# jialeli1/From-Voxel-to-Point

Measured on AMD Instinct MI355X. Metric: point clouds/sec fwd+bwd (FV2P, KITTI shape) at 1/2/4/8 MI355X, higher is better.
Workload: dtype f32

## Files before the change

### from-voxel-to-point_amd/csrc/sa_fused.hip

```cpp
#include "common.hpp"

namespace fv2p {

typedef float f32x4 __attribute__((ext_vector_type(4)));

constexpr int kSaC = 64;
constexpr int kSaCentres = 16;

__device__ __forceinline__ void row16_max_n(float (&v)[16]) {
  asm volatile(
      "s_nop 1\n\t"
      "v_max_f32_dpp %0, %0, %0 quad_perm:[1,0,3,2] row_mask:0xf bank_mask:0xf\n\t"
      "v_max_f32_dpp %1, %1, %1 quad_perm:[1,0,3,2] row_mask:0xf bank_mask:0xf\n\t"
      "v_max_f32_dpp %2, %2, %2 quad_perm:[1,0,3,2] row_mask:0xf bank_mask:0xf\n\t"
      "v_max_f32_dpp %3, %3, %3 quad_perm:[1,0,3,2] row_mask:0xf bank_mask:0xf\n\t"
      "v_max_f32_dpp %4, %4, %4 quad_perm:[1,0,3,2] row_mask:0xf bank_mask:0xf\n\t"
      "v_max_f32_dpp %5, %5, %5 quad_perm:[1,0,3,2] row_mask:0xf bank_mask:0xf\n\t"
      "v_max_f32_dpp %6, %6, %6 quad_perm:[1,0,3,2] row_mask:0xf bank_mask:0xf\n\t"
      "v_max_f32_dpp %7, %7, %7 quad_perm:[1,0,3,2] row_mask:0xf bank_mask:0xf\n\t"
      "v_max_f32_dpp %8, %8, %8 quad_perm:[1,0,3,2] row_mask:0xf bank_mask:0xf\n\t"
      "v_max_f32_dpp %9, %9, %9 quad_perm:[1,0,3,2] row_mask:0xf bank_mask:0xf\n\t"
      "v_max_f32_dpp %10, %10, %10 quad_perm:[1,0,3,2] row_mask:0xf bank_mask:0xf\n\t"
      "v_max_f32_dpp %11, %11, %11 quad_perm:[1,0,3,2] row_mask:0xf bank_mask:0xf\n\t"
      "v_max_f32_dpp %12, %12, %12 quad_perm:[1,0,3,2] row_mask:0xf bank_mask:0xf\n\t"
      "v_max_f32_dpp %13, %13, %13 quad_perm:[1,0,3,2] row_mask:0xf bank_mask:0xf\n\t"
      "v_max_f32_dpp %14, %14, %14 quad_perm:[1,0,3,2] row_mask:0xf bank_mask:0xf\n\t"
      "v_max_f32_dpp %15, %15, %15 quad_perm:[1,0,3,2] row_mask:0xf bank_mask:0xf\n\t"
      "v_max_f32_dpp %0, %0, %0 quad_perm:[2,3,0,1] row_mask:0xf bank_mask:0xf\n\t"
      "v_max_f32_dpp %1, %1, %1 quad_perm:[2,3,0,1] row_mask:0xf bank_mask:0xf\n\t"
      "v_max_f32_dpp %2, %2, %2 quad_perm:[2,3,0,1] row_mask:0xf bank_mask:0xf\n\t"
      "v_max_f32_dpp %3, %3, %3 quad_perm:[2,3,0,1] row_mask:0xf bank_mask:0xf\n\t"
      "v_max_f32_dpp %4, %4, %4 quad_perm:[2,3,0,1] row_mask:0xf bank_mask:0xf\n\t"
      "v_max_f32_dpp %5, %5, %5 quad_perm:[2,3,0,1] row_mask:0xf bank_mask:0xf\n\t"
      "v_max_f32_dpp %6, %6, %6 quad_perm:[2,3,0,1] row_mask:0xf bank_mask:0xf\n\t"
      "v_max_f32_dpp %7, %7, %7 quad_perm:[2,3,0,1] row_mask:0xf bank_mask:0xf\n\t"
      "v_max_f32_dpp %8, %8, %8 quad_perm:[2,3,0,1] row_mask:0xf bank_mask:0xf\n\t"
      "v_max_f32_dpp %9, %9, %9 quad_perm:[2,3,0,1] row_mask:0xf bank_mask:0xf\n\t"
      "v_max_f32_dpp %10, %10, %10 quad_perm:[2,3,0,1] row_mask:0xf bank_mask:0xf\n\t"
      "v_max_f32_dpp %11, %11, %11 quad_perm:[2,3,0,1] row_mask:0xf bank_mask:0xf\n\t"
      "v_max_f32_dpp %12, %12, %12 quad_perm:[2,3,0,1] row_mask:0xf bank_mask:0xf\n\t"
      "v_max_f32_dpp %13, %13, %13 quad_perm:[2,3,0,1] row_mask:0xf bank_mask:0xf\n\t"
      "v_max_f32_dpp %14, %14, %14 quad_perm:[2,3,0,1] row_mask:0xf bank_mask:0xf\n\t"
      "v_max_f32_dpp %15, %15, %15 quad_perm:[2,3,0,1] row_mask:0xf bank_mask:0xf\n\t"
      "v_max_f32_dpp %0, %0, %0 row_half_mirror row_mask:0xf bank_mask:0xf\n\t"
      "v_max_f32_dpp %1, %1, %1 row_half_mirror row_mask:0xf bank_mask:0xf\n\t"
      "v_max_f32_dpp %2, %2, %2 row_half_mirror row_mask:0xf bank_mask:0xf\n\t"
      "v_max_f32_dpp %3, %3, %3 row_half_mirror row_mask:0xf bank_mask:0xf\n\t"
      "v_max_f32_dpp %4, %4, %4 row_half_mirror row_mask:0xf bank_mask:0xf\n\t"
      "v_max_f32_dpp %5, %5, %5 row_half_mirror row_mask:0xf bank_mask:0xf\n\t"
      "v_max_f32_dpp %6, %6, %6 row_half_mirror row_mask:0xf bank_mask:0xf\n\t"
      "v_max_f32_dpp %7, %7, %7 row_half_mirror row_mask:0xf bank_mask:0xf\n\t"
      "v_max_f32_dpp %8, %8, %8 row_half_mirror row_mask:0xf bank_mask:0xf\n\t"
      "v_max_f32_dpp %9, %9, %9 row_half_mirror row_mask:0xf bank_mask:0xf\n\t"
      "v_max_f32_dpp %10, %10, %10 row_half_mirror row_mask:0xf bank_mask:0xf\n\t"
      "v_max_f32_dpp %11, %11, %11 row_half_mirror row_mask:0xf bank_mask:0xf\n\t"
      "v_max_f32_dpp %12, %12, %12 row_half_mirror row_mask:0xf bank_mask:0xf\n\t"
      "v_max_f32_dpp %13, %13, %13 row_half_mirror row_mask:0xf bank_mask:0xf\n\t"
      "v_max_f32_dpp %14, %14, %14 row_half_mirror row_mask:0xf bank_mask:0xf\n\t"
      "v_max_f32_dpp %15, %15, %15 row_half_mirror row_mask:0xf bank_mask:0xf\n\t"
      "v_max_f32_dpp %0, %0, %0 row_mirror row_mask:0xf bank_mask:0xf\n\t"
      "v_max_f32_dpp %1, %1, %1 row_mirror row_mask:0xf bank_mask:0xf\n\t"
      "v_max_f32_dpp %2, %2, %2 row_mirror row_mask:0xf bank_mask:0xf\n\t"
      "v_max_f32_dpp %3, %3, %3 row_mirror row_mask:0xf bank_mask:0xf\n\t"
      "v_max_f32_dpp %4, %4, %4 row_mirror row_mask:0xf bank_mask:0xf\n\t"
      "v_max_f32_dpp %5, %5, %5 row_mirror row_mask:0xf bank_mask:0xf\n\t"
      "v_max_f32_dpp %6, %6, %6 row_mirror row_mask:0xf bank_mask:0xf\n\t"
      "v_max_f32_dpp %7, %7, %7 row_mirror row_mask:0xf bank_mask:0xf\n\t"
      "v_max_f32_dpp %8, %8, %8 row_mirror row_mask:0xf bank_mask:0xf\n\t"
      "v_max_f32_dpp %9, %9, %9 row_mirror row_mask:0xf bank_mask:0xf\n\t"
      "v_max_f32_dpp %10, %10, %10 row_mirror row_mask:0xf bank_mask:0xf\n\t"
      "v_max_f32_dpp %11, %11, %11 row_mirror row_mask:0xf bank_mask:0xf\n\t"
      "v_max_f32_dpp %12, %12, %12 row_mirror row_mask:0xf bank_mask:0xf\n\t"
      "v_max_f32_dpp %13, %13, %13 row_mirror row_mask:0xf bank_mask:0xf\n\t"
      "v_max_f32_dpp %14, %14, %14 row_mirror row_mask:0xf bank_mask:0xf\n\t"
      "v_max_f32_dpp %15, %15, %15 row_mirror row_mask:0xf bank_mask:0xf\n\t"
      "s_nop 1"
      : "+v"(v[0]), "+v"(v[1]), "+v"(v[2]), "+v"(v[3]), "+v"(v[4]), "+v"(v[5]), "+v"(v[6]), "+v"(v[7]), "+v"(v[8]), "+v"(v[9]), "+v"(v[10]), "+v"(v[11]), "+v"(v[12]), "+v"(v[13]), "+v"(v[14]), "+v"(v[15]));
}
__device__ __forceinline__ void row16_sum_n(float (&v)[16]) {
  asm volatile(
      "s_nop 1\n\t"
      "v_add_f32_dpp %0, %0, %0 quad_perm:[1,0,3,2] row_mask:0xf bank_mask:0xf\n\t"
      "v_add_f32_dpp %1, %1, %1 quad_perm:[1,0,3,2] row_mask:0xf bank_mask:0xf\n\t"
      "v_add_f32_dpp %2, %2, %2 quad_perm:[1,0,3,2] row_mask:0xf bank_mask:0xf\n\t"
      "v_add_f32_dpp %3, %3, %3 quad_perm:[1,0,3,2] row_mask:0xf bank_mask:0xf\n\t"
      "v_add_f32_dpp %4, %4, %4 quad_perm:[1,0,3,2] row_mask:0xf bank_mask:0xf\n\t"
      "v_add_f32_dpp %5, %5, %5 quad_perm:[1,0,3,2] row_mask:0xf bank_mask:0xf\n\t"
      "v_add_f32_dpp %6, %6, %6 quad_perm:[1,0,3,2] row_mask:0xf bank_mask:0xf\n\t"
      "v_add_f32_dpp %7, %7, %7 quad_perm:[1,0,3,2] row_mask:0xf bank_mask:0xf\n\t"
      "v_add_f32_dpp %8, %8, %8 quad_perm:[1,0,3,2] row_mask:0xf bank_mask:0xf\n\t"
      "v_add_f32_dpp %9, %9, %9 quad_perm:[1,0,3,2] row_mask:0xf bank_mask:0xf\n\t"
      "v_add_f32_dpp %10, %10, %10 quad_perm:[1,0,3,2] row_mask:0xf bank_mask:0xf\n\t"
      "v_add_f32_dpp %11, %11, %11 quad_perm:[1,0,3,2] row_mask:0xf bank_mask:0xf\n\t"
      "v_add_f32_dpp %12, %12, %12 quad_perm:[1,0,3,2] row_mask:0xf bank_mask:0xf\n\t"
      "v_add_f32_dpp %13, %13, %13 quad_perm:[1,0,3,2] row_mask:0xf bank_mask:0xf\n\t"
      "v_add_f32_dpp %14, %14, %14 quad_perm:[1,0,3,2] row_mask:0xf bank_mask:0xf\n\t"
      "v_add_f32_dpp %15, %15, %15 quad_perm:[1,0,3,2] row_mask:0xf bank_mask:0xf\n\t"
      "v_add_f32_dpp %0, %0, %0 quad_perm:[2,3,0,1] row_mask:0xf bank_mask:0xf\n\t"
      "v_add_f32_dpp %1, %1, %1 quad_perm:[2,3,0,1] row_mask:0xf bank_mask:0xf\n\t"
      "v_add_f32_dpp %2, %2, %2 quad_perm:[2,3,0,1] row_mask:0xf bank_mask:0xf\n\t"
      "v_add_f32_dpp %3, %3, %3 quad_perm:[2,3,0,1] row_mask:0xf bank_mask:0xf\n\t"
      "v_add_f32_dpp %4, %4, %4 quad_perm:[2,3,0,1] row_mask:0xf bank_mask:0xf\n\t"
      "v_add_f32_dpp %5, %5, %5 quad_perm:[2,3,0,1] row_mask:0xf bank_mask:0xf\n\t"
      "v_add_f32_dpp %6, %6, %6 quad_perm:[2,3,0,1] row_mask:0xf bank_mask:0xf\n\t"
      "v_add_f32_dpp %7, %7, %7 quad_perm:[2,3,0,1] row_mask:0xf bank_mask:0xf\n\t"
      "v_add_f32_dpp %8, %8, %8 quad_perm:[2,3,0,1] row_mask:0xf bank_mask:0xf\n\t"
      "v_add_f32_dpp %9, %9, %9 quad_perm:[2,3,0,1] row_mask:0xf bank_mask:0xf\n\t"
      "v_add_f32_dpp %10, %10, %10 quad_perm:[2,3,0,1] row_mask:0xf bank_mask:0xf\n\t"
      "v_add_f32_dpp %11, %11, %11 quad_perm:[2,3,0,1] row_mask:0xf bank_mask:0xf\n\t"
      "v_add_f32_dpp %12, %12, %12 quad_perm:[2,3,0,1] row_mask:0xf bank_mask:0xf\n\t"
      "v_add_f32_dpp %13, %13, %13 quad_perm:[2,3,0,1] row_mask:0xf bank_mask:0xf\n\t"
      "v_add_f32_dpp %14, %14, %14 quad_perm:[2,3,0,1] row_mask:0xf bank_mask:0xf\n\t"
      "v_add_f32_dpp %15, %15, %15 quad_perm:[2,3,0,1] row_mask:0xf bank_mask:0xf\n\t"
      "v_add_f32_dpp %0, %0, %0 row_half_mirror row_mask:0xf bank_mask:0xf\n\t"
      "v_add_f32_dpp %1, %1, %1 row_half_mirror row_mask:0xf bank_mask:0xf\n\t"
      "v_add_f32_dpp %2, %2, %2 row_half_mirror row_mask:0xf bank_mask:0xf\n\t"
      "v_add_f32_dpp %3, %3, %3 row_half_mirror row_mask:0xf bank_mask:0xf\n\t"
      "v_add_f32_dpp %4, %4, %4 row_half_mirror row_mask:0xf bank_mask:0xf\n\t"
      "v_add_f32_dpp %5, %5, %5 row_half_mirror row_mask:0xf bank_mask:0xf\n\t"
      "v_add_f32_dpp %6, %6, %6 row_half_mirror row_mask:0xf bank_mask:0xf\n\t"
      "v_add_f32_dpp %7, %7, %7 row_half_mirror row_mask:0xf bank_mask:0xf\n\t"
      "v_add_f32_dpp %8, %8, %8 row_half_mirror row_mask:0xf bank_mask:0xf\n\t"
      "v_add_f32_dpp %9, %9, %9 row_half_mirror row_mask:0xf bank_mask:0xf\n\t"
      "v_add_f32_dpp %10, %10, %10 row_half_mirror row_mask:0xf bank_mask:0xf\n\t"
      "v_add_f32_dpp %11, %11, %11 row_half_mirror row_mask:0xf bank_mask:0xf\n\t"
      "v_add_f32_dpp %12, %12, %12 row_half_mirror row_mask:0xf bank_mask:0xf\n\t"
      "v_add_f32_dpp %13, %13, %13 row_half_mirror row_mask:0xf bank_mask:0xf\n\t"
      "v_add_f32_dpp %14, %14, %14 row_half_mirror row_mask:0xf bank_mask:0xf\n\t"
      "v_add_f32_dpp %15, %15, %15 row_half_mirror row_mask:0xf bank_mask:0xf\n\t"
      "v_add_f32_dpp %0, %0, %0 row_mirror row_mask:0xf bank_mask:0xf\n\t"
      "v_add_f32_dpp %1, %1, %1 row_mirror row_mask:0xf bank_mask:0xf\n\t"
      "v_add_f32_dpp %2, %2, %2 row_mirror row_mask:0xf bank_mask:0xf\n\t"
      "v_add_f32_dpp %3, %3, %3 row_mirror row_mask:0xf bank_mask:0xf\n\t"
      "v_add_f32_dpp %4, %4, %4 row_mirror row_mask:0xf bank_mask:0xf\n\t"
      "v_add_f32_dpp %5, %5, %5 row_mirror row_mask:0xf bank_mask:0xf\n\t"
      "v_add_f32_dpp %6, %6, %6 row_mirror row_mask:0xf bank_mask:0xf\n\t"
      "v_add_f32_dpp %7, %7, %7 row_mirror row_mask:0xf bank_mask:0xf\n\t"
      "v_add_f32_dpp %8, %8, %8 row_mirror row_mask:0xf bank_mask:0xf\n\t"
      "v_add_f32_dpp %9, %9, %9 row_mirror row_mask:0xf bank_mask:0xf\n\t"
      "v_add_f32_dpp %10, %10, %10 row_mirror row_mask:0xf bank_mask:0xf\n\t"
      "v_add_f32_dpp %11, %11, %11 row_mirror row_mask:0xf bank_mask:0xf\n\t"
      "v_add_f32_dpp %12, %12, %12 row_mirror row_mask:0xf bank_mask:0xf\n\t"
      "v_add_f32_dpp %13, %13, %13 row_mirror row_mask:0xf bank_mask:0xf\n\t"
      "v_add_f32_dpp %14, %14, %14 row_mirror row_mask:0xf bank_mask:0xf\n\t"
      "v_add_f32_dpp %15, %15, %15 row_mirror row_mask:0xf bank_mask:0xf\n\t"
      "s_nop 1"
      : "+v"(v[0]), "+v"(v[1]), "+v"(v[2]), "+v"(v[3]), "+v"(v[4]), "+v"(v[5]), "+v"(v[6]), "+v"(v[7]), "+v"(v[8]), "+v"(v[9]), "+v"(v[10]), "+v"(v[11]), "+v"(v[12]), "+v"(v[13]), "+v"(v[14]), "+v"(v[15]));
}
__device__ __forceinline__ void row16_sum_n(float (&v)[8]) {
  asm volatile(
      "s_nop 1\n\t"
      "v_add_f32_dpp %0, %0, %0 quad_perm:[1,0,3,2] row_mask:0xf bank_mask:0xf\n\t"
      "v_add_f32_dpp %1, %1, %1 quad_perm:[1,0,3,2] row_mask:0xf bank_mask:0xf\n\t"
      "v_add_f32_dpp %2, %2, %2 quad_perm:[1,0,3,2] row_mask:0xf bank_mask:0xf\n\t"
      "v_add_f32_dpp %3, %3, %3 quad_perm:[1,0,3,2] row_mask:0xf bank_mask:0xf\n\t"
      "v_add_f32_dpp %4, %4, %4 quad_perm:[1,0,3,2] row_mask:0xf bank_mask:0xf\n\t"
      "v_add_f32_dpp %5, %5, %5 quad_perm:[1,0,3,2] row_mask:0xf bank_mask:0xf\n\t"
      "v_add_f32_dpp %6, %6, %6 quad_perm:[1,0,3,2] row_mask:0xf bank_mask:0xf\n\t"
      "v_add_f32_dpp %7, %7, %7 quad_perm:[1,0,3,2] row_mask:0xf bank_mask:0xf\n\t"
      "v_add_f32_dpp %0, %0, %0 quad_perm:[2,3,0,1] row_mask:0xf bank_mask:0xf\n\t"
      "v_add_f32_dpp %1, %1, %1 quad_perm:[2,3,0,1] row_mask:0xf bank_mask:0xf\n\t"
      "v_add_f32_dpp %2, %2, %2 quad_perm:[2,3,0,1] row_mask:0xf bank_mask:0xf\n\t"
      "v_add_f32_dpp %3, %3, %3 quad_perm:[2,3,0,1] row_mask:0xf bank_mask:0xf\n\t"
      "v_add_f32_dpp %4, %4, %4 quad_perm:[2,3,0,1] row_mask:0xf bank_mask:0xf\n\t"
      "v_add_f32_dpp %5, %5, %5 quad_perm:[2,3,0,1] row_mask:0xf bank_mask:0xf\n\t"
      "v_add_f32_dpp %6, %6, %6 quad_perm:[2,3,0,1] row_mask:0xf bank_mask:0xf\n\t"
      "v_add_f32_dpp %7, %7, %7 quad_perm:[2,3,0,1] row_mask:0xf bank_mask:0xf\n\t"
      "v_add_f32_dpp %0, %0, %0 row_half_mirror row_mask:0xf bank_mask:0xf\n\t"
      "v_add_f32_dpp %1, %1, %1 row_half_mirror row_mask:0xf bank_mask:0xf\n\t"
      "v_add_f32_dpp %2, %2, %2 row_half_mirror row_mask:0xf bank_mask:0xf\n\t"
      "v_add_f32_dpp %3, %3, %3 row_half_mirror row_mask:0xf bank_mask:0xf\n\t"
      "v_add_f32_dpp %4, %4, %4 row_half_mirror row_mask:0xf bank_mask:0xf\n\t"
      "v_add_f32_dpp %5, %5, %5 row_half_mirror row_mask:0xf bank_mask:0xf\n\t"
      "v_add_f32_dpp %6, %6, %6 row_half_mirror row_mask:0xf bank_mask:0xf\n\t"
      "v_add_f32_dpp %7, %7, %7 row_half_mirror row_mask:0xf bank_mask:0xf\n\t"
      "v_add_f32_dpp %0, %0, %0 row_mirror row_mask:0xf bank_mask:0xf\n\t"
      "v_add_f32_dpp %1, %1, %1 row_mirror row_mask:0xf bank_mask:0xf\n\t"
      "v_add_f32_dpp %2, %2, %2 row_mirror row_mask:0xf bank_mask:0xf\n\t"
      "v_add_f32_dpp %3, %3, %3 row_mirror row_mask:0xf bank_mask:0xf\n\t"
      "v_add_f32_dpp %4, %4, %4 row_mirror row_mask:0xf bank_mask:0xf\n\t"
      "v_add_f32_dpp %5, %5, %5 row_mirror row_mask:0xf bank_mask:0xf\n\t"
      "v_add_f32_dpp %6, %6, %6 row_mirror row_mask:0xf bank_mask:0xf\n\t"
      "v_add_f32_dpp %7, %7, %7 row_mirror row_mask:0xf bank_mask:0xf\n\t"
      "s_nop 1"
      : "+v"(v[0]), "+v"(v[1]), "+v"(v[2]), "+v"(v[3]), "+v"(v[4]), "+v"(v[5]), "+v"(v[6]), "+v"(v[7]));
}

__device__ __forceinline__ void stage_frag(const float* __restrict__ a, bool transpose, float* __restrict__ lds) {
  for (int e = threadIdx.x; e < 16 * 64; e += blockDim.x) {
    const int lane = e & 63, bj = e >> 6, b = bj >> 2, j = bj & 3;
    const int row = 16 * b + (lane & 15), col = 16 * j + 4 * (lane >> 4);
    float4 v;
    if (!transpose) v = *reinterpret_cast<const float4*>(a + row * kSaC + col);
    else v = make_float4(a[(col + 0) * kSaC + row], a[(col + 1) * kSaC + row], a[(col + 2) * kSaC + row], a[(col + 3) * kSaC + row]);
    *reinterpret_cast<float4*>(lds + e * 4) = v;
  }
}
__device__ __forceinline__ void mma64(const float* __restrict__ frag, int lane, const float4 (&x)[4], f32x4 (&acc)[4]) {
#pragma unroll
  for (int j = 0; j < 4; ++j) {
    float4 a[4];
#pragma unroll
    for (int b = 0; b < 4; ++b) a[b] = *reinterpret_cast<const float4*>(frag + ((b * 4 + j) * 64 + lane) * 4);
#pragma unroll
    for (int b = 0; b < 4; ++b) acc[b] = __builtin_amdgcn_mfma_f32_16x16x4f32(a[b].x, x[j].x, acc[b], 0, 0, 0);
#pragma unroll
    for (int b = 0; b < 4; ++b) acc[b] = __builtin_amdgcn_mfma_f32_16x16x4f32(a[b].y, x[j].y, acc[b], 0, 0, 0);
#pragma unroll
    for (int b = 0; b < 4; ++b) acc[b] = __builtin_amdgcn_mfma_f32_16x16x4f32(a[b].z, x[j].z, acc[b], 0, 0, 0);
#pragma unroll
    for (int b = 0; b < 4; ++b) acc[b] = __builtin_amdgcn_mfma_f32_16x16x4f32(a[b].w, x[j].w, acc[b], 0, 0, 0);
  }
}
__device__ __forceinline__ float4 relu_sub(float4 p, float4 q) {
  return make_float4(fmaxf(p.x - q.x, 0.f), fmaxf(p.y - q.y, 0.f), fmaxf(p.z - q.z, 0.f), fmaxf(p.w - q.w, 0.f));
}

__global__ __launch_bounds__(256) void sa_grid_fwd_k(int n, int m, int s, const float* __restrict__ P, const float* __restrict__ Q,
                                                     const int* __restrict__ idx, const float* __restrict__ W2, float* __restrict__ out,
                                                     unsigned char* __restrict__ arg) {
  __shared__ __attribute__((aligned(16))) float wfrag[16 * 64 * 4];
  const int lane = threadIdx.x & 63, wave = threadIdx.x >> 6, row = lane & 15, g = lane >> 4;
  const int r = blockIdx.y;
  stage_frag(W2, false, wfrag);
  __syncthreads();
  const float* Pr = P + static_cast<long long>(r) * n * kSaC;
  for (int ci = wave; ci < kSaCentres; ci += 4) {
    const int i = blockIdx.x * kSaCentres + ci;
    if (i >= m) break;
    const float* q = Q + (static_cast<long long>(r) * m + i) * kSaC + 4 * g;
    float4 qv[4];
#pragma unroll
    for (int j = 0; j < 4; ++j) qv[j] = *reinterpret_cast<const float4*>(q + 16 * j);
    const int* id = idx + (static_cast<long long>(r) * m + i) * s;
    float best[4][4];
    uint32_t late = 0;
#pragma unroll
    for (int b = 0; b < 4; ++b)
#pragma unroll
      for (int e = 0; e < 4; ++e) best[b][e] = 0.f;
    for (int t = 0; t < s; t += 16) {
      const float* p = Pr + static_cast<long long>(id[t + row]) * kSaC + 4 * g;
      float4 x[4];
#pragma unroll
      for (int j = 0; j < 4; ++j) x[j] = relu_sub(*reinterpret_cast<const float4*>(p + 16 * j), qv[j]);
      f32x4 acc[4];
#pragma unroll
      for (int b = 0; b < 4; ++b) acc[b] = f32x4{0.f, 0.f, 0.f, 0.f};
      mma64(wfrag, lane, x, acc);
#pragma unroll
      for (int b = 0; b < 4; ++b)
#pragma unroll
        for (int e = 0; e < 4; ++e) {
          if (t != 0 && acc[b][e] > best[b][e]) late |= 1u << (4 * b + e);
          best[b][e] = fmaxf(best[b][e], acc[b][e]);
        }
    }
    float* o = out + (static_cast<long long>(r) * m + i) * kSaC + 4 * g;
    float flat[16];
#pragma unroll
    for (int b = 0; b < 4; ++b)
#pragma unroll
      for (int e = 0; e < 4; ++e) flat[4 * b + e] = best[b][e];
    row16_max_n(flat);
    if (row == 0) {
#pragma unroll
      for (int b = 0; b < 4; ++b) *reinterpret_cast<float4*>(o + 16 * b) = make_float4(flat[4 * b], flat[4 * b + 1], flat[4 * b + 2], flat[4 * b + 3]);
    }
    if (arg) {
      float cand[16];
#pragma unroll
      for (int k = 0; k < 16; ++k) {
        const bool holds = best[k >> 2][k & 3] == flat[k] && flat[k] > 0.f;
        cand[k] = holds ? -static_cast<float>(((late >> k) & 1u) * 16u + static_cast<uint32_t>(row)) : -255.f;
      }
      row16_max_n(cand);
      if (row == 0) {
        unsigned char* a = arg + (static_cast<long long>(r) * m + i) * kSaC + 4 * g;
#pragma unroll
        for (int b = 0; b < 4; ++b) {
          const uint32_t packed = static_cast<uint32_t>(-cand[4 * b]) | (static_cast<uint32_t>(-cand[4 * b + 1]) << 8) |
                                  (static_cast<uint32_t>(-cand[4 * b + 2]) << 16) | (static_cast<uint32_t>(-cand[4 * b + 3]) << 24);
          *reinterpret_cast<uint32_t*>(a + 16 * b) = packed;
        }
      }
    }
  }
}

constexpr int kSaTs = 72;
constexpr int kSaDp = 33;
template <int TILES, int kSaBwdWaves, bool DET>
__global__ __launch_bounds__(kSaBwdWaves * 64) void sa_grid_bwd_k(int n, int m, const float* __restrict__ P, const float* __restrict__ Q,
                                                     const int* __restrict__ idx, const float* __restrict__ W2, const unsigned char* __restrict__ arg,
                                                     const float* __restrict__ dout, float* __restrict__ dP, float* __restrict__ dQ,
                                                     float* __restrict__ dW2_partial, float* __restrict__ dh1_rows) {
  extern __shared__ __attribute__((aligned(16))) float lds[];
  float* wtfrag = lds;
  float* tile = wtfrag + 8 * 64 * 4;
  float* dpt = tile + kSaBwdWaves * 2 * 16 * kSaTs;
  const int lane = threadIdx.x & 63, wave = threadIdx.x >> 6, row = lane & 15, g = lane >> 4;
  const int half = blockIdx.x, r = blockIdx.y;
  for (int e = threadIdx.x; e < 8 * 64; e += kSaBwdWaves * 64) {
    const int l = e & 63, bj = e >> 6, bb = bj >> 2, j = bj & 3;
    const int rw = 32 * static_cast<int>(blockIdx.x) + 16 * bb + (l & 15), col = 16 * j + 4 * (l >> 4);
    *reinterpret_cast<float4*>(wtfrag + e * 4) = make_float4(W2[(col + 0) * kSaC + rw], W2[(col + 1) * kSaC + rw], W2[(col + 2) * kSaC + rw], W2[(col + 3) * kSaC + rw]);
  }
  if constexpr (!DET)
    for (int e = threadIdx.x; e < n * kSaDp; e += kSaBwdWaves * 64) dpt[e] = 0.f;
  __syncthreads();
  float* t_dh2 = tile + wave * 2 * 16 * kSaTs;
  float* t_h1 = t_dh2 + 16 * kSaTs;
  const float* Pr = P + static_cast<long long>(r) * n * kSaC;
  f32x4 dw[2][4];
#pragma unroll
  for (int bb = 0; bb < 2; ++bb)
#pragma unroll
    for (int bc = 0; bc < 4; ++bc) dw[bb][bc] = f32x4{0.f, 0.f, 0.f, 0.f};
  constexpr int s = TILES * 16;
  struct Staged { float4 qv[4], gd[4], praw[TILES][4]; uint32_t who[4]; int src[TILES]; };
  auto centre_of = [&](int i) { return static_cast<long long>(r) * m + (i < m ? i : m - 1); };
  auto load_list = [&](int i, int (&src)[TILES]) {
    const int* id = idx + centre_of(i) * s;
#pragma unroll
    for (int t = 0; t < TILES; ++t) src[t] = id[16 * t + row];
  };
  auto load_rows = [&](int i, Staged& c) {
    const long long ctr = centre_of(i);
    const float* q = Q + ctr * kSaC + 4 * g;
    const unsigned char* am = arg + ctr * kSaC + 4 * g;
    const float* go = dout + ctr * kSaC + 4 * g;
#pragma unroll
    for (int j = 0; j < 4; ++j) {
      c.qv[j] = *reinterpret_cast<const float4*>(q + 16 * j);
      c.who[j] = *reinterpret_cast<const uint32_t*>(am + 16 * j);
      c.gd[j] = *reinterpret_cast<const float4*>(go + 16 * j);
    }
#pragma unroll
    for (int t = 0; t < TILES; ++t) {
      const float* p = Pr + static_cast<long long>(c.src[t]) * kSaC + 4 * g;
#pragma unroll
      for (int j = 0; j < 4; ++j) c.praw[t][j] = *reinterpret_cast<const float4*>(p + 16 * j);
    }
  };
  Staged cur, nxt;
  int list2[TILES];
  load_list(wave, cur.src);
  load_rows(wave, cur);
  load_list(wave + kSaBwdWaves, nxt.src);
  for (int i = wave; i < m; i += kSaBwdWaves) {
    uint32_t who[4];
    float4 gd[4];
    float4 x[TILES][4];
    int src[TILES];
#pragma unroll
    for (int b = 0; b < 4; ++b) { who[b] = cur.who[b]; gd[b] = cur.gd[b]; }
#pragma unroll
    for (int t = 0; t < TILES; ++t) {
      src[t] = cur.src[t];
#pragma unroll
      for (int j = 0; j < 4; ++j) x[t][j] = relu_sub(cur.praw[t][j], cur.qv[j]);
    }
    __builtin_amdgcn_sched_barrier(0);
    load_rows(i + kSaBwdWaves, nxt);
    load_list(i + 2 * kSaBwdWaves, list2);
    __builtin_amdgcn_sched_barrier(0);
    float dq[2][4];
#pragma unroll
    for (int bb = 0; bb < 2; ++bb)
#pragma unroll
      for (int e = 0; e < 4; ++e) dq[bb][e] = 0.f;
#pragma unroll
    for (int t = 0; t < TILES; ++t) {
      float4 dh2[4];
#pragma unroll
      for (int b = 0; b < 4; ++b) {
        const float gv[4] = {gd[b].x, gd[b].y, gd[b].z, gd[b].w};
        float d[4];
#pragma unroll
        for (int e = 0; e < 4; ++e) d[e] = ((who[b] >> (8 * e)) & 0xffu) == static_cast<uint32_t>(16 * t + row) ? gv[e] : 0.f;
        dh2[b] = make_float4(d[0], d[1], d[2], d[3]);
      }
      f32x4 d1[2] = {f32x4{0.f, 0.f, 0.f, 0.f}, f32x4{0.f, 0.f, 0.f, 0.f}};
#pragma unroll
      for (int j = 0; j < 4; ++j) {
        const float4 a0 = *reinterpret_cast<const float4*>(wtfrag + ((0 * 4 + j) * 64 + lane) * 4);
        const float4 a1 = *reinterpret_cast<const float4*>(wtfrag + ((1 * 4 + j) * 64 + lane) * 4);
        d1[0] = __builtin_amdgcn_mfma_f32_16x16x4f32(a0.x, dh2[j].x, d1[0], 0, 0, 0);
        d1[1] = __builtin_amdgcn_mfma_f32_16x16x4f32(a1.x, dh2[j].x, d1[1], 0, 0, 0);
        d1[0] = __builtin_amdgcn_mfma_f32_16x16x4f32(a0.y, dh2[j].y, d1[0], 0, 0, 0);
        d1[1] = __builtin_amdgcn_mfma_f32_16x16x4f32(a1.y, dh2[j].y, d1[1], 0, 0, 0);
        d1[0] = __builtin_amdgcn_mfma_f32_16x16x4f32(a0.z, dh2[j].z, d1[0], 0, 0, 0);
        d1[1] = __builtin_amdgcn_mfma_f32_16x16x4f32(a1.z, dh2[j].z, d1[1], 0, 0, 0);
        d1[0] = __builtin_amdgcn_mfma_f32_16x16x4f32(a0.w, dh2[j].w, d1[0], 0, 0, 0);
        d1[1] = __builtin_amdgcn_mfma_f32_16x16x4f32(a1.w, dh2[j].w, d1[1], 0, 0, 0);
      }
#pragma unroll
      for (int bb = 0; bb < 2; ++bb) {
        const float4 h = half ? x[t][2 + bb] : x[t][bb];
        const float hv[4] = {h.x, h.y, h.z, h.w};
#pragma unroll
        for (int e = 0; e < 4; ++e) {
          const float v = hv[e] > 0.f ? d1[bb][e] : 0.f;
          dq[bb][e] += v;
          if constexpr (DET) dh1_rows[((static_cast<long long>(r) * m + i) * s + 16 * t + row) * kSaC + 32 * half + 16 * bb + 4 * g + e] = v;
          else if (v != 0.f) atomicAdd(&dpt[src[t] * kSaDp + 16 * bb + 4 * g + e], v);
        }
      }
#pragma unroll
      for (int b = 0; b < 4; ++b) {
        *reinterpret_cast<float4*>(t_h1 + row * kSaTs + 16 * b + 4 * g) = x[t][b];
        if ((b >> 1) == half) *reinterpret_cast<float4*>(t_dh2 + row * kSaTs + 16 * (b & 1) + 4 * g) = dh2[b];
      }
      __builtin_amdgcn_s_waitcnt(0xc07f);
#pragma unroll
      for (int ks = 0; ks < 4; ++ks) {
        float a[2], bcol[4];
#pragma unroll
        for (int bb = 0; bb < 2; ++bb) a[bb] = t_dh2[(4 * ks + g) * kSaTs + 16 * bb + row];
#pragma unroll
        for (int bc = 0; bc < 4; ++bc) bcol[bc] = t_h1[(4 * ks + g) * kSaTs + 16 * bc + row];
#pragma unroll
        for (int bb = 0; bb < 2; ++bb)
#pragma unroll
          for (int bc = 0; bc < 4; ++bc) dw[bb][bc] = __builtin_amdgcn_mfma_f32_16x16x4f32(a[bb], bcol[bc], dw[bb][bc], 0, 0, 0);
      }
    }
    float* dqo = dQ + (static_cast<long long>(r) * m + i) * kSaC + 32 * half + 4 * g;
    float flat[8];
#pragma unroll
    for (int bb = 0; bb < 2; ++bb)
#pragma unroll
      for (int e = 0; e < 4; ++e) flat[4 * bb + e] = dq[bb][e];
    row16_sum_n(flat);
    if (row == 0) {
      *reinterpret_cast<float4*>(dqo) = make_float4(-flat[0], -flat[1], -flat[2], -flat[3]);
      *reinterpret_cast<float4*>(dqo + 16) = make_float4(-flat[4], -flat[5], -flat[6], -flat[7]);
    }
    cur = nxt;
#pragma unroll
    for (int t = 0; t < TILES; ++t) nxt.src[t] = list2[t];
  }
  __syncthreads();
  float* dpo = dP + static_cast<long long>(r) * n * kSaC + 32 * half;
  for (int e = threadIdx.x; e < (DET ? 0 : n * 8); e += kSaBwdWaves * 64) {
    const int pt = e >> 3, c4 = (e & 7) * 4;
    const float* t4 = dpt + pt * kSaDp + c4;
    *reinterpret_cast<float4*>(dpo + static_cast<long long>(pt) * kSaC + c4) = make_float4(t4[0], t4[1], t4[2], t4[3]);
  }
  __syncthreads();
  float* buf = lds;
#pragma unroll
  for (int bb = 0; bb < 2; ++bb)
#pragma unroll
    for (int bc = 0; bc < 4; ++bc)
      *reinterpret_cast<f32x4*>(buf + (((wave * 2 + bb) * 4 + bc) * 64 + lane) * 4) = dw[bb][bc];
  __syncthreads();
  float* dwo = dW2_partial + (static_cast<long long>(r) * 2 + half) * 32 * kSaC;
  for (int e = threadIdx.x; e < 2 * 4 * 64 * 4; e += kSaBwdWaves * 64) {
    const int comp = e & 3, l = (e >> 2) & 63, bc = (e >> 8) & 3, bb = e >> 10;
    float v = 0.f;
#pragma unroll
    for (int w = 0; w < kSaBwdWaves; ++w) v += buf[(((w * 2 + bb) * 4 + bc) * 64 + l) * 4 + comp];
    dwo[(16 * bb + 4 * (l >> 4) + comp) * kSaC + 16 * bc + (l & 15)] = v;
  }
}

__global__ __launch_bounds__(256) void sa_grid_dw_reduce_k(int rois, const float* __restrict__ partial, float* __restrict__ dW2) {
  __shared__ float part[16][17];
  const int col = blockIdx.x * 16 + (threadIdx.x & 15), rg = threadIdx.x >> 4;
  float s = 0.f;
  for (int r = rg; r < rois; r += 16) s += partial[static_cast<long long>(r) * (kSaC * kSaC) + col];
  part[rg][threadIdx.x & 15] = s;
  __syncthreads();
  if (threadIdx.x < 16) {
    float v = part[0][threadIdx.x];
#pragma unroll
    for (int q = 1; q < 16; ++q) v += part[q][threadIdx.x];
    dW2[blockIdx.x * 16 + threadIdx.x] = v;
  }
}

}
using namespace fv2p;

static bool sa_shapes_ok(int rois, int n, int m, int s, int c) {
  return rois >= 1 && n >= 1 && m >= 1 && c == kSaC && (s == 16 || s == 32) && rois <= 65535;
}

extern "C" int fv2p_sa_grid_supported(int n, int m, int s, int c) {
  return (c == kSaC && (s == 16 || s == 32) && n >= 1 && m >= 1 && static_cast<size_t>(n) * kSaDp * 4 <= 114 * 1024) ? 1 : 0;
}

extern "C" int fv2p_sa_grid_fwd(const float* per_point, const float* per_centre, const int* idx, const float* w2, int rois, int n, int m,
                                int s, int c, float* out, unsigned char* arg, fv2p_stream_t stream) {
  FV2P_REQUIRE(sa_shapes_ok(rois, n, m, s, c), FV2P_EINVAL, "sa_grid: needs 64 channels and 16 or 32 samples per centre");
  FV2P_REQUIRE(per_point && per_centre && idx && w2 && out, FV2P_EINVAL, "sa_grid_fwd: null pointer");
  hipLaunchKernelGGL(sa_grid_fwd_k, dim3(static_cast<unsigned>(ceil_div(m, kSaCentres)), rois), dim3(256), 0, static_cast<hipStream_t>(stream),
                     n, m, s, per_point, per_centre, idx, w2, out, arg);
  FV2P_LAUNCH_CHECK();
  return 0;
}

extern "C" size_t fv2p_sa_grid_bwd_ws_bytes(int rois) {
  Sizer sz;
  sz.take<float>(static_cast<size_t>(rois > 0 ? rois : 1) * kSaC * kSaC);
  return sz.bytes();
}

template <bool DET>
static int sa_grid_bwd_launch(const float* per_point, const float* per_centre, const int* idx, const float* w2, const unsigned char* arg,
                              const float* grad_out, int rois, int n, int m, int s, float* grad_point, float* grad_centre, float* grad_w2,
                              float* partial, float* dh1_rows, hipStream_t stream) {
  auto lds_of = [&](int waves) { return (8 * 64 * 4 + static_cast<size_t>(waves) * 2 * 16 * kSaTs + static_cast<size_t>(n) * kSaDp) * sizeof(float); };
  const int waves = lds_of(8) <= 160 * 1024 ? 8 : 4;
  const size_t lds = lds_of(waves);
  static bool roomy[4] = {false, false, false, false};
  bool& raised = roomy[(s == 32 ? 2 : 0) + (waves == 8 ? 1 : 0)];
  auto launch = [&](auto kernel) -> int {
    if (lds > 48 * 1024 && !raised) {
      FV2P_HIP(hipFuncSetAttribute(reinterpret_cast<const void*>(kernel), hipFuncAttributeMaxDynamicSharedMemorySize, 160 * 1024));
      raised = true;
    }
    hipLaunchKernelGGL(kernel, dim3(2, rois), dim3(waves * 64), lds, stream, n, m, per_point, per_centre, idx, w2, arg, grad_out, grad_point, grad_centre, partial,
                       dh1_rows);
    return 0;
  };
  int rc;
  if (s == 16) rc = waves == 8 ? launch(&sa_grid_bwd_k<1, 8, DET>) : launch(&sa_grid_bwd_k<1, 4, DET>);
  else rc = waves == 8 ? launch(&sa_grid_bwd_k<2, 8, DET>) : launch(&sa_grid_bwd_k<2, 4, DET>);
  if (rc) return rc;
  hipLaunchKernelGGL(sa_grid_dw_reduce_k, dim3(kSaC * kSaC / 16), dim3(256), 0, stream, rois, partial, grad_w2);
  FV2P_LAUNCH_CHECK();
  return 0;
}

extern "C" int fv2p_sa_grid_bwd(const float* per_point, const float* per_centre, const int* idx, const float* w2, const unsigned char* arg,
                                const float* grad_out, int rois, int n, int m, int s, int c, float* grad_point, float* grad_centre,
                                float* grad_w2, void* ws, size_t ws_bytes, fv2p_stream_t stream_) {
  FV2P_REQUIRE(sa_shapes_ok(rois, n, m, s, c) && fv2p_sa_grid_supported(n, m, s, c), FV2P_EINVAL, "sa_grid_bwd: unsupported shape");
  FV2P_REQUIRE(per_point && per_centre && idx && w2 && arg && grad_out && grad_point && grad_centre && grad_w2, FV2P_EINVAL, "sa_grid_bwd: null pointer");
  FV2P_REQUIRE(ws && ws_bytes >= fv2p_sa_grid_bwd_ws_bytes(rois), FV2P_EWORKSPACE, "sa_grid_bwd: workspace too small");
  Carver cv(ws, ws_bytes);
  float* partial = cv.take<float>(static_cast<size_t>(rois) * kSaC * kSaC);
  return sa_grid_bwd_launch<false>(per_point, per_centre, idx, w2, arg, grad_out, rois, n, m, s, grad_point, grad_centre, grad_w2, partial, nullptr,
                                   static_cast<hipStream_t>(stream_));
}

__global__ void sa_grid_entries_k(int64_t entries, int n, int64_t per_roi, const int* __restrict__ idx, int* __restrict__ dst) {
  const int64_t e = static_cast<int64_t>(blockIdx.x) * blockDim.x + threadIdx.x;
  if (e >= entries) return;
  const int i = idx[e];
  dst[e] = i >= 0 && i < n ? static_cast<int>((e / per_roi) * n + i) : -1;
}

extern "C" size_t fv2p_sa_grid_bwd_gather_ws_bytes(int rois, int m, int s) {
  const int64_t entries = static_cast<int64_t>(rois > 0 ? rois : 1) * (m > 0 ? m : 1) * (s > 0 ? s : 1);
  Sizer sz;
  sz.take<char>(fv2p_sa_grid_bwd_ws_bytes(rois));
  sz.take<int>(static_cast<size_t>(entries));
  sz.take<float>(static_cast<size_t>(entries) * kSaC);
  sz.take<char>(fv2p_scatter_add_ws_bytes(entries, kSaC));
  return sz.bytes();
}

extern "C" int fv2p_sa_grid_bwd_gather(const float* per_point, const float* per_centre, const int* idx, const float* w2, const unsigned char* arg,
                                       const float* grad_out, int rois, int n, int m, int s, int c, float* grad_point, float* grad_centre,
                                       float* grad_w2, void* ws, size_t ws_bytes, fv2p_stream_t stream_) {
  hipStream_t stream = static_cast<hipStream_t>(stream_);
  FV2P_REQUIRE(sa_shapes_ok(rois, n, m, s, c) && fv2p_sa_grid_supported(n, m, s, c), FV2P_EINVAL, "sa_grid_bwd_gather: unsupported shape");
  FV2P_REQUIRE(per_point && per_centre && idx && w2 && arg && grad_out && grad_point && grad_centre && grad_w2, FV2P_EINVAL, "sa_grid_bwd_gather: null pointer");
  const int64_t entries = static_cast<int64_t>(rois) * m * s;
  FV2P_REQUIRE(entries < (1ll << 31) && static_cast<int64_t>(rois) * n < (1ll << 31) - 1, FV2P_ELIMIT, "sa_grid_bwd_gather: too many samples");
  FV2P_REQUIRE(ws && ws_bytes >= fv2p_sa_grid_bwd_gather_ws_bytes(rois, m, s), FV2P_EWORKSPACE, "sa_grid_bwd_gather: workspace too small");
  Carver cv(ws, ws_bytes);
  float* partial = reinterpret_cast<float*>(cv.take<char>(fv2p_sa_grid_bwd_ws_bytes(rois)));
  int* dst = cv.take<int>(static_cast<size_t>(entries));
  float* rows = cv.take<float>(static_cast<size_t>(entries) * kSaC);
  const size_t sb = fv2p_scatter_add_ws_bytes(entries, kSaC);
  void* sws = cv.take<char>(sb);
  if (int rc = sa_grid_bwd_launch<true>(per_point, per_centre, idx, w2, arg, grad_out, rois, n, m, s, grad_point, grad_centre, grad_w2, partial, rows,
                                        stream)) return rc;
  hipLaunchKernelGGL(sa_grid_entries_k, dim3(static_cast<unsigned>(ceil_div(entries, 256))), dim3(256), 0, stream, entries, n,
                     static_cast<int64_t>(m) * s, idx, dst);
  FV2P_HIP(hipMemsetAsync(grad_point, 0, static_cast<size_t>(rois) * n * kSaC * sizeof(float), stream));
  return fv2p_scatter_add(entries, kSaC, static_cast<int64_t>(rois) * n, dst, nullptr, nullptr, rows, 1, grad_point, sws, sb, stream);
}
```

Measured before the change: 121.9.

## Replace MFMA SA-grid backward with routed sparse scalar-indexed kernel

The non-deterministic SA grid backward path gets a new kernel. It exploits the max-pool argmax sparsity: each output channel routes gradient to only one sample, so dh1 and dW2 are built with readlane and indexed-VGPR FMAs over W2 held in registers, in place of dense MFMA tiles over all samples. Samples that no channel selected are skipped when accumulating dQ and the LDS atomics for dP. The deterministic gather path keeps the old MFMA kernel, renamed. The trade-offs are heavy inline assembly that pins fixed VGPR and SGPR ranges, a very high register footprint, and a per-sample loop that may serialize.

```diff
diff --git a/from-voxel-to-point_amd/csrc/sa_fused.hip b/from-voxel-to-point_amd/csrc/sa_fused.hip
--- a/from-voxel-to-point_amd/csrc/sa_fused.hip
+++ b/from-voxel-to-point_amd/csrc/sa_fused.hip
@@ -290,15 +290,15 @@
 
 constexpr int kSaTs = 72;
 constexpr int kSaDp = 33;
-template <int TILES, int kSaBwdWaves, bool DET>
-__global__ __launch_bounds__(kSaBwdWaves * 64) void sa_grid_bwd_k(int n, int m, const float* __restrict__ P, const float* __restrict__ Q,
+
+template <int TILES, int kSaBwdWaves>
+__global__ __launch_bounds__(kSaBwdWaves * 64) void sa_grid_bwd_rows_k(int n, int m, const float* __restrict__ P, const float* __restrict__ Q,
                                                      const int* __restrict__ idx, const float* __restrict__ W2, const unsigned char* __restrict__ arg,
-                                                     const float* __restrict__ dout, float* __restrict__ dP, float* __restrict__ dQ,
-                                                     float* __restrict__ dW2_partial, float* __restrict__ dh1_rows) {
+                                                     const float* __restrict__ dout, float* __restrict__ dQ, float* __restrict__ dW2_partial,
+                                                     float* __restrict__ dh1_rows) {
   extern __shared__ __attribute__((aligned(16))) float lds[];
   float* wtfrag = lds;
   float* tile = wtfrag + 8 * 64 * 4;
-  float* dpt = tile + kSaBwdWaves * 2 * 16 * kSaTs;
   const int lane = threadIdx.x & 63, wave = threadIdx.x >> 6, row = lane & 15, g = lane >> 4;
   const int half = blockIdx.x, r = blockIdx.y;
   for (int e = threadIdx.x; e < 8 * 64; e += kSaBwdWaves * 64) {
@@ -306,8 +306,6 @@
     const int rw = 32 * static_cast<int>(blockIdx.x) + 16 * bb + (l & 15), col = 16 * j + 4 * (l >> 4);
     *reinterpret_cast<float4*>(wtfrag + e * 4) = make_float4(W2[(col + 0) * kSaC + rw], W2[(col + 1) * kSaC + rw], W2[(col + 2) * kSaC + rw], W2[(col + 3) * kSaC + rw]);
   }
-  if constexpr (!DET)
-    for (int e = threadIdx.x; e < n * kSaDp; e += kSaBwdWaves * 64) dpt[e] = 0.f;
   __syncthreads();
   float* t_dh2 = tile + wave * 2 * 16 * kSaTs;
   float* t_h1 = t_dh2 + 16 * kSaTs;
@@ -352,15 +350,12 @@
     uint32_t who[4];
     float4 gd[4];
     float4 x[TILES][4];
-    int src[TILES];
 #pragma unroll
     for (int b = 0; b < 4; ++b) { who[b] = cur.who[b]; gd[b] = cur.gd[b]; }
 #pragma unroll
-    for (int t = 0; t < TILES; ++t) {
-      src[t] = cur.src[t];
+    for (int t = 0; t < TILES; ++t)
 #pragma unroll
       for (int j = 0; j < 4; ++j) x[t][j] = relu_sub(cur.praw[t][j], cur.qv[j]);
-    }
     __builtin_amdgcn_sched_barrier(0);
     load_rows(i + kSaBwdWaves, nxt);
     load_list(i + 2 * kSaBwdWaves, list2);
@@ -403,8 +398,7 @@
         for (int e = 0; e < 4; ++e) {
           const float v = hv[e] > 0.f ? d1[bb][e] : 0.f;
           dq[bb][e] += v;
-          if constexpr (DET) dh1_rows[((static_cast<long long>(r) * m + i) * s + 16 * t + row) * kSaC + 32 * half + 16 * bb + 4 * g + e] = v;
-          else if (v != 0.f) atomicAdd(&dpt[src[t] * kSaDp + 16 * bb + 4 * g + e], v);
+          dh1_rows[((static_cast<long long>(r) * m + i) * s + 16 * t + row) * kSaC + 32 * half + 16 * bb + 4 * g + e] = v;
         }
       }
 #pragma unroll
@@ -442,13 +436,6 @@
     for (int t = 0; t < TILES; ++t) nxt.src[t] = list2[t];
   }
   __syncthreads();
-  float* dpo = dP + static_cast<long long>(r) * n * kSaC + 32 * half;
-  for (int e = threadIdx.x; e < (DET ? 0 : n * 8); e += kSaBwdWaves * 64) {
-    const int pt = e >> 3, c4 = (e & 7) * 4;
-    const float* t4 = dpt + pt * kSaDp + c4;
-    *reinterpret_cast<float4*>(dpo + static_cast<long long>(pt) * kSaC + c4) = make_float4(t4[0], t4[1], t4[2], t4[3]);
-  }
-  __syncthreads();
   float* buf = lds;
 #pragma unroll
   for (int bb = 0; bb < 2; ++bb)
@@ -465,6 +452,135 @@
     dwo[(16 * bb + 4 * (l >> 4) + comp) * kSaC + 16 * bc + (l & 15)] = v;
   }
 }
+
+#define SA_STR_(x) #x
+#define SA_STR(x) SA_STR_(x)
+#define SA_RL(u, k0) "v_readlane_b32 s[64+2*" #u "], %[g], " SA_STR(k0) "+" #u "\n\tv_readlane_b32 s[65+2*" #u "], %[w], " SA_STR(k0) "+" #u "\n\t"
+#define SA_16(M, k0) M(0, k0) M(1, k0) M(2, k0) M(3, k0) M(4, k0) M(5, k0) M(6, k0) M(7, k0) M(8, k0) M(9, k0) M(10, k0) M(11, k0) M(12, k0) M(13, k0) M(14, k0) M(15, k0)
+#define SA_DH(u, k0) "s_set_gpr_idx_idx s[65+2*" #u "]\n\tv_fma_f32 v128, s[64+2*" #u "], v[64+" SA_STR(k0) "+" #u "], v128\n\t"
+#define SA_DH16(k0) SA_16(SA_RL, k0) "s_set_gpr_idx_on s65, gpr_idx(SRC2,DST)\n\t" SA_16(SA_DH, k0) "s_set_gpr_idx_off\n\t"
+#define SA_DW(u, k0) "s_set_gpr_idx_idx s[65+2*" #u "]\n\tv_fma_f32 %[d" #u "], s[64+2*" #u "], v160, %[d" #u "]\n\t"
+#define SA_DW16(k0) SA_16(SA_RL, k0) "s_set_gpr_idx_on s65, gpr_idx(SRC1)\n\t" SA_16(SA_DW, k0) "s_set_gpr_idx_off\n\t"
+#define SA_SGPRS "s64", "s65", "s66", "s67", "s68", "s69", "s70", "s71", "s72", "s73", "s74", "s75", "s76", "s77", "s78", "s79", "s80", "s81", "s82", "s83", \
+                 "s84", "s85", "s86", "s87", "s88", "s89", "s90", "s91", "s92", "s93", "s94", "s95"
+#define SA_DW_OPS(a, o) [d0] "+v"(a[o]), [d1] "+v"(a[o + 1]), [d2] "+v"(a[o + 2]), [d3] "+v"(a[o + 3]), [d4] "+v"(a[o + 4]), [d5] "+v"(a[o + 5]), [d6] "+v"(a[o + 6]), \
+    [d7] "+v"(a[o + 7]), [d8] "+v"(a[o + 8]), [d9] "+v"(a[o + 9]), [d10] "+v"(a[o + 10]), [d11] "+v"(a[o + 11]), [d12] "+v"(a[o + 12]), [d13] "+v"(a[o + 13]), \
+    [d14] "+v"(a[o + 14]), [d15] "+v"(a[o + 15])
+constexpr int kSaRouteWaves = 8;
+template <int S>
+__global__ __launch_bounds__(kSaRouteWaves * 64) void sa_grid_bwd_k(int n, int m, const float* __restrict__ P, const float* __restrict__ Q,
+                                                     const int* __restrict__ idx, const float* __restrict__ W2, const unsigned char* __restrict__ arg,
+                                                     const float* __restrict__ dout, float* __restrict__ dP, float* __restrict__ dQ,
+                                                     float* __restrict__ dW2_partial) {
+  typedef float rows_t __attribute__((ext_vector_type(S)));
+  extern __shared__ __attribute__((aligned(16))) float lds[];
+  float* dpt = lds;
+  const int lane = threadIdx.x & 63, wave = threadIdx.x >> 6, lc = lane & 31;
+  const int half = blockIdx.x, r = blockIdx.y;
+  const bool mine = (lane >> 5) == half;
+  typedef float w32_t __attribute__((ext_vector_type(32)));
+  w32_t w_lo, w_hi;
+#pragma unroll
+  for (int k = 0; k < 32; ++k) { w_lo[k] = W2[k * kSaC + lane]; w_hi[k] = W2[(32 + k) * kSaC + lane]; }
+  for (int e = threadIdx.x; e < n * kSaDp; e += kSaRouteWaves * 64) dpt[e] = 0.f;
+  __syncthreads();
+  const float* Pr = P + static_cast<long long>(r) * n * kSaC + lane;
+  float dw[32];
+#pragma unroll
+  for (int j = 0; j < 32; ++j) dw[j] = 0.f;
+  struct Staged { rows_t rows; float q, gd; uint32_t who; int lst; };
+  auto centre_of = [&](int i) { return static_cast<long long>(r) * m + (i < m ? i : m - 1); };
+  auto load_list = [&](int i) { return idx[centre_of(i) * S + (lane & (S - 1))]; };
+  auto load_rows = [&](int i, Staged& c) {
+    const long long ctr = centre_of(i);
+    c.q = Q[ctr * kSaC + lane];
+    c.who = arg[ctr * kSaC + lane];
+    c.gd = dout[ctr * kSaC + lane];
+    const int inside = min(max(c.lst, 0), n - 1);
+#pragma unroll
+    for (int s = 0; s < S; ++s) c.rows[s] = Pr[static_cast<long long>(__builtin_amdgcn_readlane(inside, s)) * kSaC];
+  };
+  Staged cur, nxt;
+  cur.lst = load_list(wave);
+  load_rows(wave, cur);
+  nxt.lst = load_list(wave + kSaRouteWaves);
+  for (int i = wave; i < m; i += kSaRouteWaves) {
+    rows_t h;
+#pragma unroll
+    for (int s = 0; s < S; ++s) h[s] = fmaxf(cur.rows[s] - cur.q, 0.f);
+    asm volatile("" : "+v"(h));
+    bool live = cur.who < static_cast<uint32_t>(S);
+    const int list = cur.lst;
+    const int pt = __builtin_amdgcn_ds_bpermute(live ? static_cast<int>(cur.who << 2) : 0, list);
+    live = live && static_cast<uint32_t>(pt) < static_cast<uint32_t>(n);
+    const int g_lane = live ? static_cast<int>(__float_as_uint(cur.gd)) : 0, who_lane = live ? static_cast<int>(cur.who) : 0;
+    int bits = live ? 1 << cur.who : 0;
+    bits |= __builtin_amdgcn_update_dpp(0, bits, 0xb1, 0xf, 0xf, false);
+    bits |= __builtin_amdgcn_update_dpp(0, bits, 0x4e, 0xf, 0xf, false);
+    bits |= __builtin_amdgcn_update_dpp(0, bits, 0x141, 0xf, 0xf, false);
+    bits |= __builtin_amdgcn_update_dpp(0, bits, 0x140, 0xf, 0xf, false);
+    const uint32_t routed = static_cast<uint32_t>(__builtin_amdgcn_readlane(bits, 0) | __builtin_amdgcn_readlane(bits, 16) |
+                                                  __builtin_amdgcn_readlane(bits, 32) | __builtin_amdgcn_readlane(bits, 48));
+    __builtin_amdgcn_sched_barrier(0);
+    load_rows(i + kSaRouteWaves, nxt);
+    const int list2 = load_list(i + 2 * kSaRouteWaves);
+    __builtin_amdgcn_sched_barrier(0);
+    rows_t dh1;
+#pragma unroll
+    for (int s = 0; s < S; ++s) dh1[s] = 0.f;
+    if constexpr (S == 32)
+      asm volatile(SA_DH16(0) SA_DH16(16) SA_DH16(32) SA_DH16(48) : "+{v[128:159]}"(dh1) : [g] "v"(g_lane), [w] "v"(who_lane), "{v[64:95]}"(w_lo), "{v[96:127]}"(w_hi) : SA_SGPRS);
+    else
+      asm volatile(SA_DH16(0) SA_DH16(16) SA_DH16(32) SA_DH16(48) : "+{v[128:143]}"(dh1) : [g] "v"(g_lane), [w] "v"(who_lane), "{v[64:95]}"(w_lo), "{v[96:127]}"(w_hi) : SA_SGPRS);
+    const int g_half = __builtin_amdgcn_ds_bpermute((32 * half + lc) << 2, g_lane), who_half = __builtin_amdgcn_ds_bpermute((32 * half + lc) << 2, who_lane);
+    if constexpr (S == 32) {
+      asm volatile(SA_DW16(0) : SA_DW_OPS(dw, 0) : [g] "v"(g_half), [w] "v"(who_half), "{v[160:191]}"(h) : SA_SGPRS);
+      asm volatile(SA_DW16(16) : SA_DW_OPS(dw, 16) : [g] "v"(g_half), [w] "v"(who_half), "{v[160:191]}"(h) : SA_SGPRS);
+    } else {
+      asm volatile(SA_DW16(0) : SA_DW_OPS(dw, 0) : [g] "v"(g_half), [w] "v"(who_half), "{v[160:175]}"(h) : SA_SGPRS);
+      asm volatile(SA_DW16(16) : SA_DW_OPS(dw, 16) : [g] "v"(g_half), [w] "v"(who_half), "{v[160:175]}"(h) : SA_SGPRS);
+    }
+    float dq = 0.f;
+#pragma unroll
+    for (int s = 0; s < S; ++s) {
+      if (!(routed & (1u << s))) continue;
+      const float v = h[s] > 0.f ? dh1[s] : 0.f;
+      dq += v;
+      if (mine && v != 0.f) atomicAdd(&dpt[__builtin_amdgcn_readlane(list, s) * kSaDp + lc], v);
+    }
+    if (mine) dQ[(static_cast<long long>(r) * m + i) * kSaC + lane] = -dq;
+    cur = nxt;
+    nxt.lst = list2;
+  }
+  __syncthreads();
+  float* dpo = dP + static_cast<long long>(r) * n * kSaC + 32 * half;
+  for (int e = threadIdx.x; e < n * 8; e += kSaRouteWaves * 64) {
+    const int pt = e >> 3, ch = (e & 7) * 4;
+    const float* t4 = dpt + pt * kSaDp + ch;
+    *reinterpret_cast<float4*>(dpo + static_cast<long long>(pt) * kSaC + ch) = make_float4(t4[0], t4[1], t4[2], t4[3]);
+  }
+  __syncthreads();
+#pragma unroll
+  for (int j = 0; j < 32; ++j) lds[(wave * 32 + j) * kSaC + lane] = dw[j];
+  __syncthreads();
+  float* dwo = dW2_partial + (static_cast<long long>(r) * 2 + half) * 32 * kSaC;
+  for (int e = threadIdx.x; e < 32 * kSaC; e += kSaRouteWaves * 64) {
+    float v = 0.f;
+#pragma unroll
+    for (int w = 0; w < kSaRouteWaves; ++w) v += lds[w * 32 * kSaC + e];
+    dwo[e] = v;
+  }
+}
+#undef SA_STR_
+#undef SA_STR
+#undef SA_RL
+#undef SA_16
+#undef SA_DH
+#undef SA_DH16
+#undef SA_DW
+#undef SA_DW16
+#undef SA_SGPRS
+#undef SA_DW_OPS
 
 __global__ __launch_bounds__(256) void sa_grid_dw_reduce_k(int rois, const float* __restrict__ partial, float* __restrict__ dW2) {
   __shared__ float part[16][17];
@@ -508,27 +624,45 @@
   return sz.bytes();
 }
 
-template <bool DET>
+template <typename Kernel, typename... Args>
+static int sa_grid_bwd_launch_one(Kernel kernel, bool& raised, int rois, int waves, size_t lds, hipStream_t stream, Args... args) {
+  if (lds > 48 * 1024 && !raised) {
+    FV2P_HIP(hipFuncSetAttribute(reinterpret_cast<const void*>(kernel), hipFuncAttributeMaxDynamicSharedMemorySize, 160 * 1024));
+    raised = true;
+  }
+  hipLaunchKernelGGL(kernel, dim3(2, rois), dim3(waves * 64), lds, stream, args...);
+  return 0;
+}
+
 static int sa_grid_bwd_launch(const float* per_point, const float* per_centre, const int* idx, const float* w2, const unsigned char* arg,
                               const float* grad_out, int rois, int n, int m, int s, float* grad_point, float* grad_centre, float* grad_w2,
-                              float* partial, float* dh1_rows, hipStream_t stream) {
-  auto lds_of = [&](int waves) { return (8 * 64 * 4 + static_cast<size_t>(waves) * 2 * 16 * kSaTs + static_cast<size_t>(n) * kSaDp) * sizeof(float); };
-  const int waves = lds_of(8) <= 160 * 1024 ? 8 : 4;
+                              float* partial, hipStream_t stream) {
+  const size_t tile = static_cast<size_t>(n) * kSaDp * sizeof(float), fold = static_cast<size_t>(kSaRouteWaves) * 32 * kSaC * sizeof(float);
+  const size_t lds = tile > fold ? tile : fold;
+  static bool roomy[2] = {false, false};
+  auto launch = [&](auto kernel, bool& raised) {
+    return sa_grid_bwd_launch_one(kernel, raised, rois, kSaRouteWaves, lds, stream, n, m, per_point, per_centre, idx, w2, arg, grad_out, grad_point, grad_centre, partial);
+  };
+  if (int rc = s == 16 ? launch(&sa_grid_bwd_k<16>, roomy[0]) : launch(&sa_grid_bwd_k<32>, roomy[1])) return rc;
+  hipLaunchKernelGGL(sa_grid_dw_reduce_k, dim3(kSaC * kSaC / 16), dim3(256), 0, stream, rois, partial, grad_w2);
+  FV2P_LAUNCH_CHECK();
+  return 0;
+}
+
+static int sa_grid_bwd_rows_launch(const float* per_point, const float* per_centre, const int* idx, const float* w2, const unsigned char* arg,
+                                   const float* grad_out, int rois, int n, int m, int s, float* grad_centre, float* grad_w2, float* partial,
+                                   float* dh1_rows, hipStream_t stream) {
+  auto lds_of = [&](int waves) { return (8 * 64 * 4 + static_cast<size_t>(waves) * 2 * 16 * kSaTs) * sizeof(float); };
+  const int waves = lds_of(8) + static_cast<size_t>(n) * kSaDp * sizeof(float) <= 160 * 1024 ? 8 : 4;
   const size_t lds = lds_of(waves);
   static bool roomy[4] = {false, false, false, false};
   bool& raised = roomy[(s == 32 ? 2 : 0) + (waves == 8 ? 1 : 0)];
-  auto launch = [&](auto kernel) -> int {
-    if (lds > 48 * 1024 && !raised) {
-      FV2P_HIP(hipFuncSetAttribute(reinterpret_cast<const void*>(kernel), hipFuncAttributeMaxDynamicSharedMemorySize, 160 * 1024));
-      raised = true;
-    }
-    hipLaunchKernelGGL(kernel, dim3(2, rois), dim3(waves * 64), lds, stream, n, m, per_point, per_centre, idx, w2, arg, grad_out, grad_point, grad_centre, partial,
-                       dh1_rows);
-    return 0;
+  auto launch = [&](auto kernel) {
+    return sa_grid_bwd_launch_one(kernel, raised, rois, waves, lds, stream, n, m, per_point, per_centre, idx, w2, arg, grad_out, grad_centre, partial, dh1_rows);
   };
   int rc;
-  if (s == 16) rc = waves == 8 ? launch(&sa_grid_bwd_k<1, 8, DET>) : launch(&sa_grid_bwd_k<1, 4, DET>);
-  else rc = waves == 8 ? launch(&sa_grid_bwd_k<2, 8, DET>) : launch(&sa_grid_bwd_k<2, 4, DET>);
+  if (s == 16) rc = waves == 8 ? launch(&sa_grid_bwd_rows_k<1, 8>) : launch(&sa_grid_bwd_rows_k<1, 4>);
+  else rc = waves == 8 ? launch(&sa_grid_bwd_rows_k<2, 8>) : launch(&sa_grid_bwd_rows_k<2, 4>);
   if (rc) return rc;
   hipLaunchKernelGGL(sa_grid_dw_reduce_k, dim3(kSaC * kSaC / 16), dim3(256), 0, stream, rois, partial, grad_w2);
   FV2P_LAUNCH_CHECK();
@@ -543,8 +677,8 @@
   FV2P_REQUIRE(ws && ws_bytes >= fv2p_sa_grid_bwd_ws_bytes(rois), FV2P_EWORKSPACE, "sa_grid_bwd: workspace too small");
   Carver cv(ws, ws_bytes);
   float* partial = cv.take<float>(static_cast<size_t>(rois) * kSaC * kSaC);
-  return sa_grid_bwd_launch<false>(per_point, per_centre, idx, w2, arg, grad_out, rois, n, m, s, grad_point, grad_centre, grad_w2, partial, nullptr,
-                                   static_cast<hipStream_t>(stream_));
+  return sa_grid_bwd_launch(per_point, per_centre, idx, w2, arg, grad_out, rois, n, m, s, grad_point, grad_centre, grad_w2, partial,
+                            static_cast<hipStream_t>(stream_));
 }
 
 __global__ void sa_grid_entries_k(int64_t entries, int n, int64_t per_roi, const int* __restrict__ idx, int* __restrict__ dst) {
@@ -579,8 +713,7 @@
   float* rows = cv.take<float>(static_cast<size_t>(entries) * kSaC);
   const size_t sb = fv2p_scatter_add_ws_bytes(entries, kSaC);
   void* sws = cv.take<char>(sb);
-  if (int rc = sa_grid_bwd_launch<true>(per_point, per_centre, idx, w2, arg, grad_out, rois, n, m, s, grad_point, grad_centre, grad_w2, partial, rows,
-                                        stream)) return rc;
+  if (int rc = sa_grid_bwd_rows_launch(per_point, per_centre, idx, w2, arg, grad_out, rois, n, m, s, grad_centre, grad_w2, partial, rows, stream)) return rc;
   hipLaunchKernelGGL(sa_grid_entries_k, dim3(static_cast<unsigned>(ceil_div(entries, 256))), dim3(256), 0, stream, entries, n,
                      static_cast<int64_t>(m) * s, idx, dst);
   FV2P_HIP(hipMemsetAsync(grad_point, 0, static_cast<size_t>(rois) * n * kSaC * sizeof(float), stream));
```

After: 122.5 (median of 5 runs). About the same (+0.5%).
